# phymhan/pc-gan

Measured on AMD Instinct MI355X. Metric: images/sec (G+D step) 128x128 bs32 per GPU, higher is better.
Workload: dtype f32; 1 GPU; wsgan_emb UTKFace-shaped 128x128 bs32/GPU fp32: 9-block ResnetGenerator + 3-layer PatchGAN + ResNet-18 Elo encoder@224 + AlexNet IP@224, full optimize_parameters(); global_batch=32, parallelism=dp1

## Files before the change

pc-gan_amd/csrc/hgemm.hip:

```cpp
#include "igemm.h"

namespace pcgan {

typedef _Float16 f16x8 __attribute__((ext_vector_type(8)));
typedef _Float16 f16x4 __attribute__((ext_vector_type(4)));

typedef __bf16 bf16x8v __attribute__((ext_vector_type(8)));
typedef __bf16 bf16x4v __attribute__((ext_vector_type(4)));

template <int MODE, int BM, int BP, typename TA>
__global__ void __launch_bounds__(256) hgemm_kernel(IgemmArgs a) {
    static_assert(MODE == MODE_FWD_ZERO || MODE == MODE_FWD_REFLECT || MODE == MODE_BWD, "forward and plain data gradient");
    constexpr bool HALF = sizeof(TA) == 2;
    constexpr int NP = HALF ? 1 : 2;
    constexpr unsigned ES = sizeof(TA);
    constexpr int WM = (BM == 128 || (BM == 64 && BP == 64)) ? 2 : 1;
    constexpr int WP = 4 / WM;
    constexpr int WMT = BM / WM, WPT = BP / WP;
    constexpr int MI = WMT / 32, PJ = WPT / 32;
    constexpr int KPT = BP / 16;
    constexpr int ACH = BM * 4 / 256;
    constexpr int TROWS = NTAP_FWD + 1;
    constexpr int AH = BM + 8;
    __shared__ __attribute__((aligned(16))) f16x8 As[2][NP][2 * AH];
    __shared__ __attribute__((aligned(16))) f16x8 Bs[2][NP][2 * BP];
    __shared__ unsigned offT[TROWS][BP];
    __shared__ __attribute__((aligned(16))) float biasS[BM];
    __shared__ __attribute__((aligned(16))) float iswS[BM];

    const int nMt = (a.M + BM - 1) / BM;
    const int mt = blockIdx.x % nMt;
    int pt = blockIdx.x / nMt;
    int phase = 0;
    while (phase + 1 < a.nphase && pt >= a.tstart[phase + 1]) ++phase;
    pt -= a.tstart[phase];
    const PhaseArgs& P = a.ph[phase];
    const int tid = threadIdx.x;
    const int lane = tid & 63, lo = lane & 31, hi = lane >> 5;
    const int wave = __builtin_amdgcn_readfirstlane(tid >> 6);
    const int wm = wave / WP, wp = wave % WP;
    const int Ptot = P.Ptot, Kp = P.Kp;
    const int m0 = mt * BM, p0 = pt * BP;
    const int ph_nS = P.nS;
    const int T = P.nR * ph_nS;
    const int HgWg4 = a.Hg * a.Wg * (int)ES;
    const __amdgpu_buffer_rsrc_t rX = make_rsrc(a.X, a.x_bytes);
    const __amdgpu_buffer_rsrc_t rA = make_rsrc(P.A, (unsigned)a.M * (unsigned)Kp * 4u);

    float sx = 1.f;
    const int pl = tid % BP;
    {
        const int pg = p0 + pl;
        const bool pvalid = pg < Ptot;
        int gn = 0, py = 0, px = 0;
        if (pvalid) pix_coord(a, P, pg, gn, py, px);
        const unsigned vbase = (unsigned)gn * (unsigned)a.Cg * (unsigned)(a.Hg * a.Wg);
        for (int t = tid / BP; t <= T; t += 256 / BP) {
            const int ri = t / ph_nS, sj = t - ri * ph_nS;
            const int r = P.r0 + ri * a.tstep, sxx = P.s0 + sj * a.tstep;
            const bool live = pvalid && t < T;
            const unsigned y = axis_entry<MODE>(py, py + a.pad, true, r, a.Hg, a.sl, a.pad);
            const unsigned x = axis_entry<MODE>(px, px + a.pad, true, sxx, a.Wg, a.sl, a.pad);
            offT[t][pl] = (live && y != 0xffffffffu && x != 0xffffffffu) ? (vbase + y * (unsigned)a.Wg + x) * ES : OOB;
        }
    }
    const int ksub = __builtin_amdgcn_readfirstlane(tid / BP);
    __syncthreads();

    const int nst_all = Kp >> 4;
    const int nst_per = a.ksplit > 1 ? (nst_all + a.ksplit - 1) / a.ksplit : nst_all;
    const int st_begin = a.ksplit > 1 ? (int)blockIdx.z * nst_per : 0;
    const int st_end = st_begin + nst_per < nst_all ? st_begin + nst_per : nst_all;
    const int nst_here = st_end > st_begin ? st_end - st_begin : 0;

    int it_tap, it_c, it_k0, it_left = nst_here;
    {
        const int cc0 = st_begin / T;
        it_tap = st_begin - cc0 * T;
        it_c = cc0 * 16;
        it_k0 = st_begin * 16;
    }
    unsigned a_base[ACH];
#pragma unroll
    for (int j = 0; j < ACH; ++j) {
        const int q = tid + 256 * j;
        const int row = q >> 2, kc = (q & 3) * 4;
        a_base[j] = (m0 + row < a.M) ? (unsigned)((m0 + row) * Kp + kc) * 4u : OOB;
    }
    struct Stage {
        u32x4 av[ACH];
        unsigned bv[KPT];
    };
    auto load = [&](Stage& r) {
        const bool live = it_left > 0;
        const unsigned vo = offT[live ? it_tap : T][pl];
        const unsigned so = (unsigned)((it_c + ksub * KPT) * HgWg4);
#pragma unroll
        for (int j = 0; j < ACH; ++j) r.av[j] = __builtin_amdgcn_raw_buffer_load_b128(rA, live ? a_base[j] : OOB, (unsigned)it_k0 * 4u, 0);
#pragma unroll
        for (int i = 0; i < KPT; ++i) {
            if constexpr (HALF) r.bv[i] = (unsigned)__builtin_amdgcn_raw_buffer_load_b16(rX, vo, so + (unsigned)(i * HgWg4), 0);
            else r.bv[i] = __builtin_amdgcn_raw_buffer_load_b32(rX, vo, so + (unsigned)(i * HgWg4), 0);
        }
        --it_left;
        const int t1 = it_tap + 1;
        const bool wr = t1 == T;
        it_tap = wr ? 0 : t1;
        it_c += wr ? 16 : 0;
        it_k0 += 16;
    };
    auto stash = [&](const Stage& r, int buf) {
        if constexpr (HALF) {
#pragma unroll
            for (int j = 0; j < ACH; ++j) {
                const int q = tid + 256 * j;
                const int row = q >> 2, kc = (q & 3) * 4;
                bf16x4v h;
#pragma unroll
                for (int e = 0; e < 4; ++e) h[e] = (__bf16)__uint_as_float(r.av[j][e]);
                *reinterpret_cast<bf16x4v*>(reinterpret_cast<__bf16*>(&As[buf][0][(kc >> 3) * AH + row]) + (kc & 4)) = h;
            }
            typedef unsigned short usK __attribute__((ext_vector_type(KPT)));
            usK v;
#pragma unroll
            for (int e = 0; e < KPT; ++e) v[e] = (unsigned short)r.bv[e];
            if constexpr (KPT == 8) *reinterpret_cast<usK*>(&Bs[buf][0][ksub * BP + pl]) = v;
            else *reinterpret_cast<usK*>(reinterpret_cast<unsigned short*>(&Bs[buf][0][(ksub >> 1) * BP + pl]) + (ksub & 1) * 4) = v;
            return;
        }
#pragma unroll
        for (int j = 0; j < ACH; ++j) {
            const int q = tid + 256 * j;
            const int row = q >> 2, kc = (q & 3) * 4;
            typedef unsigned u32x2 __attribute__((ext_vector_type(2)));
            u32x2 h, l;
            h[0] = r.av[j][0]; h[1] = r.av[j][1];
            l[0] = r.av[j][2]; l[1] = r.av[j][3];
            _Float16* d0 = reinterpret_cast<_Float16*>(&As[buf][0][(kc >> 3) * AH + row]) + (kc & 4);
            _Float16* d1 = reinterpret_cast<_Float16*>(&As[buf][NP - 1][(kc >> 3) * AH + row]) + (kc & 4);
            *reinterpret_cast<u32x2*>(d0) = h;
            *reinterpret_cast<u32x2*>(d1) = l;
        }
        if constexpr (KPT == 8) {
            f16x8 h, l;
#pragma unroll
            for (int e = 0; e < 8; ++e) {
                _Float16 x, y;
                split2h(__uint_as_float(r.bv[e]) * sx, x, y);
                h[e] = x;
                l[e] = y;
            }
            Bs[buf][0][ksub * BP + pl] = h;
            Bs[buf][NP - 1][ksub * BP + pl] = l;
        } else {
            f16x4 h, l;
#pragma unroll
            for (int e = 0; e < 4; ++e) {
                _Float16 x, y;
                split2h(__uint_as_float(r.bv[e]) * sx, x, y);
                h[e] = x;
                l[e] = y;
            }
            *reinterpret_cast<f16x4*>(reinterpret_cast<_Float16*>(&Bs[buf][0][(ksub >> 1) * BP + pl]) + (ksub & 1) * 4) = h;
            *reinterpret_cast<f16x4*>(reinterpret_cast<_Float16*>(&Bs[buf][NP - 1][(ksub >> 1) * BP + pl]) + (ksub & 1) * 4) = l;
        }
    };

    f32x16 acc[MI][PJ];
#pragma unroll
    for (int i = 0; i < MI; ++i)
#pragma unroll
        for (int j = 0; j < PJ; ++j)
#pragma unroll
            for (int r = 0; r < 16; ++r) acc[i][j][r] = 0.f;
    struct Operands {
        f16x8 A[NP][MI], B[NP][PJ];
    };
    auto fetch = [&](Operands& o, int buf) {
#pragma unroll
        for (int p = 0; p < NP; ++p) {
#pragma unroll
            for (int i = 0; i < MI; ++i) o.A[p][i] = As[buf][p][hi * AH + wm * WMT + i * 32 + lo];
#pragma unroll
            for (int j = 0; j < PJ; ++j) o.B[p][j] = Bs[buf][p][hi * BP + wp * WPT + j * 32 + lo];
        }
    };
    auto mma = [&](const Operands& o) {
        if constexpr (HALF) {
#pragma unroll
            for (int i = 0; i < MI; ++i)
#pragma unroll
                for (int j = 0; j < PJ; ++j)
                    acc[i][j] = __builtin_amdgcn_mfma_f32_32x32x16_bf16(__builtin_bit_cast(bf16x8v, o.A[0][i]), __builtin_bit_cast(bf16x8v, o.B[0][j]),
                                                                         acc[i][j], 0, 0, 0);
            return;
        }
        constexpr int PA[3] = {NP - 1, 0, 0}, PB[3] = {0, NP - 1, 0};
#pragma unroll
        for (int q = 0; q < 3; ++q)
#pragma unroll
            for (int i = 0; i < MI; ++i)
#pragma unroll
                for (int j = 0; j < PJ; ++j)
                    acc[i][j] = __builtin_amdgcn_mfma_f32_32x32x16_f16(o.A[PA[q]][i], o.B[PB[q]][j], acc[i][j], 0, 0, 0);
    };
    auto interleave = [&]() {
        constexpr int NM = (HALF ? 1 : 3) * MI * PJ, NRD = NP * (MI + PJ);
#pragma unroll
        for (int q = 0; q < NM; ++q) {
            __builtin_amdgcn_sched_group_barrier(0x008, 1, 0);
            __builtin_amdgcn_sched_group_barrier(0x100, (NRD + NM - 1) / NM, 0);
            __builtin_amdgcn_sched_group_barrier(0x002, 48 / NM + 1, 0);
            __builtin_amdgcn_sched_group_barrier(0x200, 1, 0);
            __builtin_amdgcn_sched_group_barrier(0x020, (ACH + KPT + NM - 1) / NM, 0);
        }
    };

    Stage rg[2];
    if (nst_here > 0) {
        load(rg[0]);
        load(rg[1]);
    }
    if constexpr (!HALF) {
        const float m = thread_max_of_partials(a.x_amax, a.x_namax, tid, 256);
        sx = pow2_scale(block_max(m, biasS));
// ... 6 lines not shown
        Operands op[2];
        stash(rg[0], 0);
        __syncthreads();
        load(rg[0]);
        fetch(op[0], 0);
        stash(rg[1], 1);
        __syncthreads();
        load(rg[1]);
        const int nst2 = (nst_here + 1) & ~1;
        for (int s = 0; s < nst2; s += 2) {
#pragma unroll
            for (int t = 0; t < 2; ++t) {
                fetch(op[t ^ 1], t ^ 1);
                mma(op[t]);
                stash(rg[t], t);
                load(rg[t]);
                interleave();
                __builtin_amdgcn_sched_barrier(0);
                __syncthreads();
                __builtin_amdgcn_sched_barrier(0);
            }
        }
    }

    const float isx = 1.f / sx;
    const int YhYw = a.Yh * a.Yw;
    bool bad = false;
    if constexpr (!HALF) {
#pragma unroll
        for (int j = 0; j < PJ; ++j)
#pragma unroll
            for (int i = 0; i < MI; ++i)
#pragma unroll
                for (int r = 0; r < 16; ++r) bad |= is_nonfinite(acc[i][j][r]);
        report_nonfinite(a.ovf, bad);
    }
#pragma unroll
    for (int j = 0; j < PJ; ++j) {
        const int pix = p0 + wp * WPT + j * 32 + lo;
        if (pix >= Ptot) continue;
        int n, oy, ox;
        pix_coord(a, P, pix, n, oy, ox);
        if (a.ksplit > 1) {
            float* Yp = a.Ypart + ((size_t)blockIdx.z * a.N + n) * a.M * YhYw + oy * a.Yw + ox;
#pragma unroll
            for (int i = 0; i < MI; ++i)
#pragma unroll
                for (int r = 0; r < 16; ++r) {
                    const int ml = wm * WMT + i * 32 + (r & 3) + 8 * (r >> 2) + 4 * hi;
                    const int m = m0 + ml;
                    if (m < a.M) Yp[(size_t)m * YhYw] = (acc[i][j][r] * isx) * (HALF ? 1.f : iswS[ml]);
                }
            continue;
        }
        TA* Yp = (TA*)a.Y + (size_t)n * a.M * YhYw + oy * a.Yw + ox;
#pragma unroll
        for (int i = 0; i < MI; ++i)
#pragma unroll
            for (int r = 0; r < 16; ++r) {
                const int ml = wm * WMT + i * 32 + (r & 3) + 8 * (r >> 2) + 4 * hi;
                if (m0 + ml < a.M) st1(Yp + (size_t)(m0 + ml) * YhYw, act_apply((acc[i][j][r] * isx) * (HALF ? 1.f : iswS[ml]) + biasS[ml], a.act, a.slope));
            }
    }
}

template <int MODE>
static void launch_mode(const IgemmArgs& a, int bm, int bp, dim3 grid2, hipStream_t st) {
    if (bm == 128 && bp == 128) LAUNCH_TA(a.dtype, hgemm_kernel, grid2, a, MODE, 128, 128);
    else if (bm == 128) LAUNCH_TA(a.dtype, hgemm_kernel, grid2, a, MODE, 128, 64);
    else if (bp == 128) LAUNCH_TA(a.dtype, hgemm_kernel, grid2, a, MODE, 64, 128);
    else LAUNCH_TA(a.dtype, hgemm_kernel, grid2, a, MODE, 64, 64);
}
int launch_hgemm(int mode, const IgemmArgs& a, int bm, int bp, dim3 grid2, hipStream_t st) {
    switch (mode) {
        case MODE_FWD_ZERO: launch_mode<MODE_FWD_ZERO>(a, bm, bp, grid2, st); break;
        case MODE_FWD_REFLECT: launch_mode<MODE_FWD_REFLECT>(a, bm, bp, grid2, st); break;
        case MODE_BWD: launch_mode<MODE_BWD>(a, bm, bp, grid2, st); break;
        default: PCGAN_CHECK(false, "hgemm: no kernel for mode %d", mode);
    }
    PCGAN_LAUNCH_CHECK();
    return 0;
}

}

using namespace pcgan;

__global__ void __launch_bounds__(256) hgemm_presplit_kernel(float* __restrict__ A, int M, int Kp4, const float* __restrict__ rowmax) {
    const size_t n4 = (size_t)M * Kp4;
    for (size_t i = (size_t)blockIdx.x * 256 + threadIdx.x; i < n4; i += (size_t)gridDim.x * 256) {
        const float s = pow2_scale(rowmax[i / Kp4]);
        const float4 v = reinterpret_cast<const float4*>(A)[i];
        f16x4 h, l;
        _Float16 x, y;
        split2h(v.x * s, x, y); h[0] = x; l[0] = y;
        split2h(v.y * s, x, y); h[1] = x; l[1] = y;
        split2h(v.z * s, x, y); h[2] = x; l[2] = y;
        split2h(v.w * s, x, y); h[3] = x; l[3] = y;
        reinterpret_cast<f16x4*>(A)[2 * i] = h;
        reinterpret_cast<f16x4*>(A)[2 * i + 1] = l;
    }
}

int pcgan::launch_hgemm_presplit(float* A, int M, int Kp4, const float* rowmax, hipStream_t st) {
    hipLaunchKernelGGL(hgemm_presplit_kernel, dim3(capped_blocks((size_t)M * Kp4, 256, 2048)), dim3(256), 0, st, A, M, Kp4, rowmax);
    PCGAN_LAUNCH_CHECK();
    return 0;
}
```

pc-gan_amd/csrc/igemm.h:

```cpp
#pragma once
#include "common.h"
#include <type_traits>

namespace pcgan {

typedef float f32x16 __attribute__((ext_vector_type(16)));

enum { MODE_FWD_ZERO = 0, MODE_FWD_REFLECT = 1, MODE_BWD = 2, MODE_BWD_REFLECT = 3 };

typedef unsigned int u32x4 __attribute__((ext_vector_type(4)));
static constexpr unsigned OOB = 0x80000000u;

__device__ __forceinline__ __amdgpu_buffer_rsrc_t make_rsrc(const void* p, unsigned bytes) {
    return __builtin_amdgcn_make_buffer_rsrc(const_cast<void*>(p), 0, (int)bytes, 0x00020000);
}
__device__ __forceinline__ float ld_b32(__amdgpu_buffer_rsrc_t r, unsigned voff, unsigned soff) {
    return __uint_as_float(__builtin_amdgcn_raw_buffer_load_b32(r, voff, soff, 0));
}
__device__ __forceinline__ float4 ld_b128(__amdgpu_buffer_rsrc_t r, unsigned voff) {
    const u32x4 v = __builtin_amdgcn_raw_buffer_load_b128(r, voff, 0, 0);
    return make_float4(__uint_as_float(v.x), __uint_as_float(v.y), __uint_as_float(v.z), __uint_as_float(v.w));
}

template <typename TA>
// ... 115 lines not shown

struct Geom {
    int Hg, Wg, sl, pad;
};

template <int MODE>
__device__ __forceinline__ bool tap_offset(const Geom& a, int py, int px, int r, int s, int& off) {
    if (MODE == MODE_BWD || MODE == MODE_BWD_REFLECT) {
        const int ty = py + a.pad - r, tx = px + a.pad - s;
        const int oy = ty >> a.sl, ox = tx >> a.sl;
        off = oy * a.Wg + ox;
        return (ty >= 0) & (tx >= 0) & (oy < a.Hg) & (ox < a.Wg);
    } else {
        int iy = (py << a.sl) - a.pad + r;
        int ix = (px << a.sl) - a.pad + s;
        if (MODE == MODE_FWD_REFLECT) {
            iy = iy < 0 ? -iy : iy;
            iy = iy >= a.Hg ? 2 * (a.Hg - 1) - iy : iy;
            ix = ix < 0 ? -ix : ix;
            ix = ix >= a.Wg ? 2 * (a.Wg - 1) - ix : ix;
            off = iy * a.Wg + ix;
            return true;
        } else {
            off = iy * a.Wg + ix;
            return ((unsigned)iy < (unsigned)a.Hg) & ((unsigned)ix < (unsigned)a.Wg);
        }
    }
}

struct KIter {
    int ri, sj, c;
    __device__ __forceinline__ void advance(int n, int Cgp, int nS) {
        c += n;
        while (c >= Cgp) {
            c -= Cgp;
            if (++sj == nS) {
                sj = 0;
                ++ri;
            }
        }
    }
};

static constexpr int NTAP_FWD = 25;
static constexpr int NTAP_MIR = 9;
static constexpr int NTAP_CG4 = 49;

template <int MODE>
__device__ __forceinline__ unsigned axis_entry(int p, int base, bool base_ok, int tap, int n, int sl, int pad) {
    int i;
    bool ok;
    if (MODE == MODE_BWD || MODE == MODE_BWD_REFLECT) {
        const int t = base - tap;
        i = t >> sl;
        ok = base_ok & (t >= 0) & (i < n);
    } else {
        i = (p << sl) - pad + tap;
        if (MODE == MODE_FWD_REFLECT) {
            i = i < 0 ? -i : i;
            i = i >= n ? 2 * (n - 1) - i : i;
            ok = true;
        } else {
            ok = (unsigned)i < (unsigned)n;
        }
    }
    return ok ? (unsigned)i : 0xffffffffu;
}

__device__ __forceinline__ float4 ld_b128s(__amdgpu_buffer_rsrc_t r, unsigned voff, unsigned soff) {
    const u32x4 v = __builtin_amdgcn_raw_buffer_load_b128(r, voff, soff, 0);
    return make_float4(__uint_as_float(v.x), __uint_as_float(v.y), __uint_as_float(v.z), __uint_as_float(v.w));
}

__device__ __forceinline__ int refl_inner(int i, int n, int p) { return i == 0 ? 0 : (i == n - 2 * p - 1 ? n - 1 : i + p); }
__device__ __forceinline__ void pix_coord(const IgemmArgs& a, const PhaseArgs& P, int pg, int& n, int& py, int& px) {
    const int HsWs = P.Hs * P.Ws;
    n = pg / HsWs;
    const int rem = pg - n * HsWs;
    const int sy = rem / P.Ws;
    py = P.ymap ? refl_inner(sy, a.Yh, a.pad) : sy * a.ostep + P.fy;
    px = (rem - sy * P.Ws) * a.ostep + P.fx;
}

struct WgradArgs {
    const void* dY;
    const void* X;
    int dtype;
    float* Wp;
    int M, Kp, N, Cg, Cgp, Hg, Wg, Ho, Wo;
    int sl, pad, S;
    int magicS;
    int Ptot, chunks_per_split;
    unsigned x_bytes, dy_bytes;
};

static constexpr unsigned SM_INV = 0x40000000u;

static inline int round4(int v) { return (v + 3) & ~3; }
static inline size_t esz(const pcgan_conv_desc* d) { return d->dtype == PCGAN_BF16 ? 2 : 4; }

#define LAUNCH_TA(dt, KERNEL, GRID, ARG, ...)                                                                   \
    do {                                                                                                        \
        if ((dt) == PCGAN_BF16) hipLaunchKernelGGL((KERNEL<__VA_ARGS__, bf16>), GRID, dim3(256), 0, st, ARG);    \
        else hipLaunchKernelGGL((KERNEL<__VA_ARGS__, float>), GRID, dim3(256), 0, st, ARG);                      \
    } while (0)

void record_launch(int form, int mode, int bm, int bp, int ks, int nphase);
int launch_splitk_reduce(int dtype, hipStream_t st, const float* part, void* y, const float* bias, int ks, size_t out_elems, int M,
                         int HW, int act, float slope);

int launch_igemm_f32(int mode, const IgemmArgs& a, int bm, int bp, dim3 grid, dim3 grid2, hipStream_t st);
int launch_hgemm(int mode, const IgemmArgs& a, int bm, int bp, dim3 grid2, hipStream_t st);
int launch_hgemm_presplit(float* A, int M, int Kp4, const float* rowmax, hipStream_t st);
int launch_smallm(int mode, IgemmArgs& a, int pmax, hipStream_t st, float* part_ws, size_t part_bytes);
int launch_transpose4(const float* A, float* At, int M, int Kp, hipStream_t st);
int launch_pack_strip(const float* A, float* Ws, int M, int Cg, int Cgp, int nR, int nS, hipStream_t st);
int wgrad_splits(const pcgan_conv_desc* d, int* chunks_per_split);
int launch_wgrad(const pcgan_conv_desc* d, const WgradArgs& a, int splits, float* dw, int accumulate, hipStream_t st);

}
```

pc-gan_amd/csrc/igemm_conv.hip:

```cpp
#include "igemm.h"
#include <stdlib.h>
#include <mutex>

namespace pcgan {

template <typename TA>
__global__ void splitk_reduce_kernel(const float* __restrict__ part, TA* __restrict__ y, const float* __restrict__ bias,
                                     int ks, size_t n, int M, int HW, int act, float slope) {
    const size_t n4 = (n & 3) ? 0 : (n >> 2);
    const size_t stride = (size_t)gridDim.x * blockDim.x;
    for (size_t i = blockIdx.x * (size_t)blockDim.x + threadIdx.x; i < n4; i += stride) {
        float4 acc = reinterpret_cast<const float4*>(part)[i];
        for (int s = 1; s < ks; ++s) {
            const float4 v = reinterpret_cast<const float4*>(part + (size_t)s * n)[i];
            acc.x += v.x; acc.y += v.y; acc.z += v.z; acc.w += v.w;
        }
        float o[4] = {acc.x, acc.y, acc.z, acc.w};
#pragma unroll
        for (int u = 0; u < 4; ++u) {
            const size_t e = i * 4 + u;
            if (bias) o[u] += bias[(e / HW) % M];
            o[u] = act_apply(o[u], act, slope);
        }
        st4(y + 4 * i, make_float4(o[0], o[1], o[2], o[3]));
    }
    for (size_t e = (n4 << 2) + blockIdx.x * (size_t)blockDim.x + threadIdx.x; e < n; e += stride) {
        float acc = 0.f;
        for (int s = 0; s < ks; ++s) acc += part[(size_t)s * n + e];
        if (bias) acc += bias[(e / HW) % M];
        st1(y + e, act_apply(acc, act, slope));
    }
}

__global__ void repack_fwd_kernel(const float* __restrict__ w, float* __restrict__ A, int K, int C, int Cgp,
                                  int RS, int chunked) {
    const int Kp = RS * Cgp;
    const size_t total = (size_t)K * Kp;
    for (size_t i = blockIdx.x * (size_t)blockDim.x + threadIdx.x; i < total; i += (size_t)gridDim.x * blockDim.x) {
        const int k = (int)(i / Kp);
        const int j = (int)(i - (size_t)k * Kp);
        int tap, c;
        if (chunked) {
            const int t2 = j >> 4;
            const int cc = t2 / RS;
            tap = t2 - cc * RS;
            c = cc * 16 + (j & 15);
        } else {
            tap = j / Cgp;
            c = j - tap * Cgp;
        }
        A[i] = (c < C) ? w[((size_t)k * C + c) * RS + tap] : 0.f;
    }
}
__global__ void repack_bwd_kernel(const float* __restrict__ w, float* __restrict__ A, int K, int C, int Kgp,
                                  int R, int S, int r0, int s0, int tstep, int nR, int nS, int chunked, int fold) {
    const int Kp = nR * nS * Kgp;
    const size_t total = (size_t)C * Kp;
    for (size_t i = blockIdx.x * (size_t)blockDim.x + threadIdx.x; i < total; i += (size_t)gridDim.x * blockDim.x) {
        const int c = (int)(i / Kp);
        const int j = (int)(i - (size_t)c * Kp);
        int t, k;
        if (chunked) {
            const int t2 = j >> 4;
            const int kc = t2 / (nR * nS);
            t = t2 - kc * (nR * nS);
            k = kc * 16 + (j & 15);
        } else {
            t = j / Kgp;
            k = j - t * Kgp;
        }
        const int ri = t / nS, sj = t - ri * nS;
        const int r = r0 + ri * tstep, s = s0 + sj * tstep;
        float v = (k < K) ? w[(((size_t)k * C + c) * R + r) * S + s] : 0.f;
        if (k < K && fold == 1 && r == R - 1) v += w[(((size_t)k * C + c) * R + 0) * S + s];
        if (k < K && fold == 2 && r == 0) v += w[(((size_t)k * C + c) * R + (R - 1)) * S + s];
        A[i] = v;
    }
}

struct PackBwdArgs {
    const float* w;
    int K, C, Kgp, R, S, tstep, chunked, n;
    struct Entry {
        float* A;
        int r0, s0, nR, nS, fold;
    } e[16];
};
__global__ void repack_bwd_multi_kernel(PackBwdArgs a) {
    const PackBwdArgs::Entry& E = a.e[blockIdx.y];
    const int RS = E.nR * E.nS;
    const int Kp = RS * a.Kgp;
    const size_t total = (size_t)a.C * Kp;
    for (size_t i = blockIdx.x * (size_t)blockDim.x + threadIdx.x; i < total; i += (size_t)gridDim.x * blockDim.x) {
        const int c = (int)(i / Kp);
        const int j = (int)(i - (size_t)c * Kp);
        int t, k;
        if (a.chunked) {
            const int t2 = j >> 4;
            const int kc = t2 / RS;
            t = t2 - kc * RS;
            k = kc * 16 + (j & 15);
        } else {
            t = j / a.Kgp;
            k = j - t * a.Kgp;
        }
        const int ri = t / E.nS, sj = t - ri * E.nS;
        const int r = E.r0 + ri * a.tstep, sx = E.s0 + sj * a.tstep;
        float v = 0.f;
        if (k < a.K) {
            const float* wk = a.w + ((size_t)k * a.C + c) * a.R * a.S;
            v = wk[r * a.S + sx];
            if (E.fold == 1 && r == a.R - 1) v += wk[sx];
            if (E.fold == 2 && r == 0) v += wk[(a.R - 1) * a.S + sx];
        }
        E.A[i] = v;
    }
}

template <typename TA>
__global__ void reflect_fold_kernel(const TA* __restrict__ t, TA* __restrict__ dx, int NC, int H, int W,
                                    int pad, const float* __restrict__ bias, int C) {
    const int Hp = H + 2 * pad, Wp = W + 2 * pad;
    const int W4 = (W + 3) >> 2;
    const TA* tp = t + (size_t)blockIdx.y * Hp * Wp;
    TA* dp = dx + (size_t)blockIdx.y * H * W;
    const float bv = bias ? bias[blockIdx.y % C] : 0.f;
    for (int i = blockIdx.x * blockDim.x + threadIdx.x; i < H * W4; i += gridDim.x * blockDim.x) {
        const int y = i / W4, x0 = (i - y * W4) * 4;
        int ys[3], ny = 0;
        ys[ny++] = y + pad;
        if (y >= 1 && y <= pad) ys[ny++] = pad - y;
        if (y >= H - 1 - pad && y <= H - 2) ys[ny++] = pad + 2 * (H - 1) - y;
        float acc[4] = {0.f, 0.f, 0.f, 0.f};
        for (int a = 0; a < ny; ++a) {
            const TA* row = tp + ys[a] * Wp;
#pragma unroll
            for (int j = 0; j < 4; ++j) {
                const int x = x0 + j;
                if (x >= W) continue;
                float v = ld1(row + x + pad);
                if (x >= 1 && x <= pad) v += ld1(row + pad - x);
                if (x >= W - 1 - pad && x <= W - 2) v += ld1(row + pad + 2 * (W - 1) - x);
                acc[j] += v;
            }
        }
        if (bias) {
#pragma unroll
            for (int j = 0; j < 4; ++j) acc[j] += bv;
        }
        if ((W & 3) == 0) {
            st4(dp + y * W + x0, make_float4(acc[0], acc[1], acc[2], acc[3]));
        } else {
            for (int j = 0; j < 4 && x0 + j < W; ++j) st1(dp + y * W + x0 + j, acc[j]);
        }
    }
}

int launch_splitk_reduce(int dtype, hipStream_t st, const float* part, void* y, const float* bias, int ks, size_t out_elems, int M,
                         int HW, int act, float slope) {
    const dim3 b(capped_blocks(out_elems / 4, 256, 4096));
    if (dtype == PCGAN_BF16)
        hipLaunchKernelGGL(splitk_reduce_kernel<bf16>, b, dim3(256), 0, st, part, (bf16*)y, bias, ks, out_elems, M, HW, act, slope);
    else
        hipLaunchKernelGGL(splitk_reduce_kernel<float>, b, dim3(256), 0, st, part, (float*)y, bias, ks, out_elems, M, HW, act, slope);
    PCGAN_LAUNCH_CHECK();
    return 0;
}

static int check_desc(const pcgan_conv_desc* d) {
    PCGAN_CHECK(d != nullptr, "conv: null descriptor");
    PCGAN_CHECK(d->N > 0 && d->C > 0 && d->H > 0 && d->W > 0 && d->K > 0 && d->R > 0 && d->S > 0,
                "conv: non-positive dimension");
    PCGAN_CHECK(ilog2_exact(d->stride) >= 0 && d->stride <= 4, "conv: stride %d unsupported (1,2,4)", d->stride);
    PCGAN_CHECK(d->pad_mode == 0 || d->pad_mode == 1, "conv: pad_mode %d", d->pad_mode);
    PCGAN_CHECK(d->dtype == PCGAN_F32 || d->dtype == PCGAN_BF16, "conv: dtype %d (PCGAN_F32 / PCGAN_BF16)", d->dtype);
    const int P = (d->H + 2 * d->pad - d->R) / d->stride + 1, Q = (d->W + 2 * d->pad - d->S) / d->stride + 1;
    PCGAN_CHECK(P == d->P && Q == d->Q, "conv: output dims %dx%d do not match geometry %dx%d", d->P, d->Q, P, Q);
    if (d->pad_mode == 1)
        PCGAN_CHECK(d->pad < d->H && d->pad < d->W, "conv: reflection pad %d >= input size", d->pad);
    const size_t xin = (size_t)d->N * d->C * (d->H + 2 * d->pad) * (d->W + 2 * d->pad) * 4;
    const size_t yout = (size_t)d->N * d->K * d->P * d->Q * 4;
    PCGAN_CHECK(xin < (1ull << 31) && yout < (1ull << 31),
                "conv: tensor of %zu bytes exceeds the 2 GiB addressing limit of one launch (split the batch)",
                xin > yout ? xin : yout);
    PCGAN_CHECK((size_t)d->K * round4(d->C) * d->R * d->S * 4 < (1ull << 31) &&
                    (size_t)d->C * round4(d->K) * d->R * d->S * 4 < (1ull << 31), "conv: weight tensor too large");
    PCGAN_CHECK(d->R * d->S <= 512, "conv: filter too large");
    return 0;
}

static inline bool chunked_k(int Cg, int M, int R, int S) { return (Cg % 16) == 0 && M > 4 && R * S <= NTAP_FWD; }
static inline bool cg4_k(int Cg, int M, int R, int S) { return round4(Cg) == 4 && M > 4 && R * S <= NTAP_CG4; }
static inline long tile_blocks(int M, int ptot_max, int nphase, int mm, int pp) {
    return (long)((M + mm - 1) / mm) * ((ptot_max + pp - 1) / pp) * nphase;
}
static inline long split_below() { return 192; }
static inline bool may_split(int M, int ptot_max, int nphase) {
    if (option(OPT_HGEMM_KS) > 1) return M > 4;
// ... 221 lines not shown
}

struct BwdPhase {
    int fy, fx, r0, s0, nR, nS, Hs, Ws;
    int fold;
    size_t a_off, at_off, as_off;
};
struct BwdPlan {
    bool fused, rowfold, padded;
    int H, W, pad;
    bool need_zero;
    int n;
    BwdPhase ph[16];
};
static void bwd_plan(const pcgan_conv_desc* d, BwdPlan& pl) {
    memset(&pl, 0, sizeof(pl));
    pl.fused = bwd_fused_reflect(d);
    pl.rowfold = bwd_rowfold(d);
    pl.padded = d->pad_mode == 1 && !pl.fused;
    const int H = pl.H = pl.padded ? d->H + 2 * d->pad : d->H;
    const int W = pl.W = pl.padded ? d->W + 2 * d->pad : d->W;
    const int pad = pl.pad = pl.padded ? 0 : d->pad;
    const int stv = d->stride, Kgp = round4(d->K), RS = d->R * d->S;
    if (pl.rowfold) {
        for (int f = 0; f < 3; ++f) {
            BwdPhase& p = pl.ph[pl.n++];
            p.nR = d->R; p.nS = d->S; p.Ws = W; p.fold = f;
            p.Hs = f == 0 ? H - 2 : 1;
            p.fy = f == 0 ? 0 : (f == 1 ? 1 : H - 2);
            p.a_off = (size_t)f * d->C * RS * Kgp;
        }
        return;
    }
    size_t a_off = 0;
    size_t at_off = (size_t)d->C * RS * Kgp;
    size_t as_off = at_off + (size_t)RS * Kgp * 4;
    for (int fy = 0; fy < stv; ++fy) {
        for (int fx = 0; fx < stv; ++fx) {
            const int r0 = (fy + pad) % stv, s0 = (fx + pad) % stv;
            const int nR = r0 < d->R ? (d->R - r0 + stv - 1) / stv : 0;
            const int nS = s0 < d->S ? (d->S - s0 + stv - 1) / stv : 0;
            const int Hs = fy < H ? (H - fy + stv - 1) / stv : 0;
            const int Ws = fx < W ? (W - fx + stv - 1) / stv : 0;
            if (Hs * Ws == 0) continue;
            if (nR * nS == 0) {
                pl.need_zero = true;
                continue;
            }
            const BwdPhase p = {fy, fx, r0, s0, nR, nS, Hs, Ws, 0, a_off, at_off, as_off};
            pl.ph[pl.n++] = p;
            a_off += (size_t)d->C * nR * nS * Kgp;
            at_off += (size_t)nR * nS * Kgp * 4;
            as_off += (size_t)d->K * nS * 32;
        }
    }
}

static int pack_bwd(const pcgan_conv_desc* d, const BwdPlan& pl, const float* w, float* packed, hipStream_t st) {
    const int Kgp = round4(d->K);
    const int chunked = (int)chunked_k(d->K, d->C, d->R, d->S);
    if (d->C <= 4) {
        for (int i = 0; i < pl.n; ++i) {
            const BwdPhase& p = pl.ph[i];
            float* A = packed + p.a_off;
            const size_t total = (size_t)d->C * p.nR * p.nS * Kgp;
            hipLaunchKernelGGL(repack_bwd_kernel, dim3(capped_blocks(total, 256, 4096)), dim3(256), 0, st, w, A, d->K, d->C, Kgp, d->R,
                               d->S, p.r0, p.s0, d->stride, p.nR, p.nS, chunked, 0);
            PCGAN_LAUNCH_CHECK();
            if (int e = launch_transpose4(A, packed + p.at_off, d->C, p.nR * p.nS * Kgp, st)) return e;
            if (int e = launch_pack_strip(A, packed + p.as_off, d->C, d->K, Kgp, p.nR, p.nS, st)) return e;
        }
        return 0;
    }
    if (pl.n == 0) return 0;
    size_t max_total = 0;
    PackBwdArgs pk;
    memset(&pk, 0, sizeof(pk));
    pk.w = w; pk.K = d->K; pk.C = d->C; pk.Kgp = Kgp; pk.R = d->R; pk.S = d->S; pk.tstep = d->stride; pk.chunked = chunked; pk.n = pl.n;
    for (int i = 0; i < pl.n; ++i) {
        const BwdPhase& p = pl.ph[i];
        const size_t total = (size_t)d->C * p.nR * p.nS * Kgp;
        max_total = total > max_total ? total : max_total;
        PackBwdArgs::Entry& pe = pk.e[i];
        pe.A = packed + p.a_off; pe.r0 = p.r0; pe.s0 = p.s0; pe.nR = p.nR; pe.nS = p.nS; pe.fold = p.fold;
    }
    hipLaunchKernelGGL(repack_bwd_multi_kernel, dim3(capped_blocks(max_total, 256, 2048), pk.n), dim3(256), 0, st, pk);
    PCGAN_LAUNCH_CHECK();
    return 0;
}

static int conv2d_bwd_data_impl(const pcgan_conv_desc* d, const void* dy, const float* w, const float* packed,
                                const float* bias, void* dx, void* ws, size_t ws_bytes, pcgan_stream_t s, const HsplitOpt* hs = nullptr) {
    if (check_desc(d)) return 1;
    PCGAN_CHECK(dy && (w || packed), "conv2d_bwd_data: null pointer");
    PCGAN_CHECK(ws && ws_bytes >= pcgan_conv2d_workspace_bytes(d, PCGAN_PASS_BWD_DATA),
                "conv2d_bwd_data: workspace too small (%zu)", ws_bytes);
    PCGAN_CHECK(d->pad_mode == 0 || d->stride == 1, "conv2d_bwd_data: reflection padding needs stride 1");
    hipStream_t st = (hipStream_t)s;
    const int Kgp = round4(d->K), stv = d->stride;
    BwdPlan pl;
    bwd_plan(d, pl);
    float* Abase = packed ? const_cast<float*>(packed) : (float*)ws;
    if (!packed && pack_bwd(d, pl, w, Abase, st)) return 2;
    const size_t a_bytes = bwd_base_bytes(d);
    const int H = pl.H, W = pl.W;
    void* out = pl.padded ? (void*)((char*)ws + a_bytes) : dx;

    IgemmArgs a;
    memset(&a, 0, sizeof(a));
    a.X = dy; a.Y = out; a.dtype = d->dtype;
    a.bias = pl.padded ? nullptr : bias;
    a.M = d->C; a.N = d->N; a.Cg = d->K; a.Cgp = Kgp; a.Hg = d->P; a.Wg = d->Q;
    a.Yh = H; a.Yw = W;
    a.ostep = stv; a.sl = ilog2_exact(stv); a.pad = pl.pad; a.tstep = stv;
    a.act = PCGAN_ACT_NONE; a.slope = 0.f;
    a.chunked = chunked_k(d->K, d->C, d->R, d->S) ? 1 : (cg4_k(d->K, d->C, d->R, d->S) ? 2 : 0);
    a.rowfold = pl.rowfold;
    apply_hsplit(a, hs);
    a.x_bytes = (unsigned)((size_t)d->N * d->K * d->P * d->Q * esz(d));
    a.nphase = pl.n;
    for (int i = 0; i < pl.n; ++i) {
        const BwdPhase& q = pl.ph[i];
        PhaseArgs& p = a.ph[i];
        p.A = Abase + q.a_off; p.Kp = q.nR * q.nS * Kgp; p.Hs = q.Hs; p.Ws = q.Ws; p.fy = q.fy; p.fx = q.fx;
        if (d->C <= 4) {
            p.A = Abase + q.at_off;
            p.As = Abase + q.as_off;
        }
        p.r0 = q.r0; p.s0 = q.s0; p.nR = q.nR; p.nS = q.nS; p.Ptot = d->N * q.Hs * q.Ws;
        p.ymap = pl.rowfold && q.fold == 0;
    }
    if (pl.rowfold) return launch_igemm(MODE_BWD_REFLECT, a, st, nullptr, 0);
    if (pl.need_zero) {
        PCGAN_CHECK(!bias, "conv2d_bwd_data: bias with uncovered phases is unsupported");
        hipError_t e = hipMemsetAsync(out, 0, (size_t)d->N * d->C * H * W * esz(d), st);
        PCGAN_CHECK(e == hipSuccess, "memset failed: %s", hipGetErrorString(e));
    }
    float* part = (bwd_part_bytes(d) && !pl.padded && !pl.need_zero) ? (float*)((char*)ws + a_bytes) : nullptr;
    if (launch_igemm(pl.fused ? MODE_BWD_REFLECT : MODE_BWD, a, st, part, bwd_part_bytes(d))) return 2;
    if (pl.padded) return pcgan::launch_reflect_fold(out, dx, d->N * d->C, d->H, d->W, d->pad, d->dtype, st, bias, d->C);
    return 0;
}

extern "C" int pcgan_conv2d_bwd_data(const pcgan_conv_desc* d, const void* dy, const float* w,
                                     const float* bias, void* dx, void* ws, size_t ws_bytes,
                                     pcgan_stream_t s) {
    if (check_desc(d)) return 1;
    PCGAN_CHECK(w && dx, "conv2d_bwd_data: null pointer");
    return conv2d_bwd_data_impl(d, dy, w, nullptr, bias, dx, ws, ws_bytes, s);
}
extern "C" int pcgan_conv2d_bwd_data_packed(const pcgan_conv_desc* d, const void* dy, const float* packed,
                                            const float* bias, void* dx, void* ws, size_t ws_bytes,
                                            pcgan_stream_t s) {
    if (check_desc(d)) return 1;
    PCGAN_CHECK(packed && dx, "conv2d_bwd_data_packed: null pointer");
    pcgan::TimerScope timer(pcgan::timer_kind_res(d, pcgan::TIMER_RES_DGRAD), (hipStream_t)s);
    return conv2d_bwd_data_impl(d, dy, nullptr, packed, bias, dx, ws, ws_bytes, s);
}

extern "C" int pcgan_conv2d_hgemm_supported(const pcgan_conv_desc* d, int pass) {
    if (!d || d->dtype != PCGAN_F32) return 0;
    if (pass == PCGAN_PASS_FWD) return chunked_k(d->C, d->K, d->R, d->S) && d->K > 32;
    if (pass == PCGAN_PASS_BWD_DATA) return d->pad_mode == 0 && chunked_k(d->K, d->C, d->R, d->S) && d->C > 32;
    return 0;
}
extern "C" int pcgan_conv2d_fwd_packed_hsplit(const pcgan_conv_desc* d, const void* x, const float* x_amax, int n_amax, const float* packed,
                                              const float* w_amax, const float* bias, void* y, int act, float slope, void* ws,
                                              size_t ws_bytes, pcgan_stream_t s) {
    if (check_desc(d)) return 1;
    PCGAN_CHECK(pcgan_conv2d_hgemm_supported(d, PCGAN_PASS_FWD), "conv2d_fwd_packed_hsplit: unsupported shape");
    PCGAN_CHECK(packed && x_amax && n_amax > 0 && w_amax, "conv2d_fwd_packed_hsplit: null pointer");
    const HsplitOpt hs = {x_amax, n_amax, w_amax};
    return conv2d_fwd_impl(d, x, nullptr, packed, bias, y, act, slope, ws, ws_bytes, s, &hs);
}
extern "C" int pcgan_conv2d_bwd_data_packed_hsplit(const pcgan_conv_desc* d, const void* dy, const float* dy_amax, int n_amax,
                                                   const float* packed, const float* w_amax, const float* bias, void* dx, void* ws,
                                                   size_t ws_bytes, pcgan_stream_t s) {
    if (check_desc(d)) return 1;
    PCGAN_CHECK(pcgan_conv2d_hgemm_supported(d, PCGAN_PASS_BWD_DATA), "conv2d_bwd_data_packed_hsplit: unsupported shape");
    PCGAN_CHECK(packed && dx && dy_amax && n_amax > 0 && w_amax, "conv2d_bwd_data_packed_hsplit: null pointer");
    const HsplitOpt hs = {dy_amax, n_amax, w_amax};
    return conv2d_bwd_data_impl(d, dy, nullptr, packed, bias, dx, ws, ws_bytes, s, &hs);
}

extern "C" int pcgan_conv2d_hgemm_pack(const pcgan_conv_desc* d, int pass, const float* w, float* w_rowmax, float* packed,
                                       pcgan_stream_t s) {
    if (check_desc(d)) return 1;
    PCGAN_CHECK(pcgan_conv2d_hgemm_supported(d, pass), "conv2d_hgemm_pack: unsupported shape or pass");
    PCGAN_CHECK(w && w_rowmax && packed, "conv2d_hgemm_pack: null pointer");
    hipStream_t st = (hipStream_t)s;
    const bool fwd = pass == PCGAN_PASS_FWD;
    const int M = fwd ? d->K : d->C, RS = d->R * d->S;
    if (launch_weight_row_absmax(w, d->K, d->C, RS, fwd ? 0 : 1, w_rowmax, st)) return 2;
    if (pcgan_conv2d_pack_weights(d, pass, w, packed, s)) return 1;
    if (fwd) return launch_hgemm_presplit(packed, M, RS * round4(d->C) / 4, w_rowmax, st);
    BwdPlan pl;
    bwd_plan(d, pl);
    for (int i = 0; i < pl.n; ++i)
        if (int e = launch_hgemm_presplit(packed + pl.ph[i].a_off, M, pl.ph[i].nR * pl.ph[i].nS * round4(d->K) / 4, w_rowmax, st)) return e;
    return 0;
}

extern "C" int pcgan_igemm_last_launch(int* info, int n) {
    PCGAN_CHECK(info != nullptr && n > 0, "igemm_last_launch: null output");
    std::lock_guard<std::mutex> lk(g_launch_mu);
    for (int i = 0; i < n; ++i) info[i] = i < PCGAN_IGEMM_LAUNCH_INFO ? g_launch[i] : 0;
    return 0;
}

extern "C" size_t pcgan_conv2d_packed_bytes(const pcgan_conv_desc* d, int pass) {
    if (!d) return 0;
    if (pass == PCGAN_PASS_FWD) return fwd_base_bytes(d);
    if (pass == PCGAN_PASS_BWD_DATA) return bwd_base_bytes(d);
    return 0;
}
extern "C" int pcgan_conv2d_pack_weights(const pcgan_conv_desc* d, int pass, const float* w, float* packed,
                                         pcgan_stream_t s) {
    if (check_desc(d)) return 1;
    PCGAN_CHECK(w && packed, "conv2d_pack_weights: null pointer");
    if (pass == PCGAN_PASS_FWD) return pack_fwd(d, w, packed, (hipStream_t)s);
    PCGAN_CHECK(pass == PCGAN_PASS_BWD_DATA, "conv2d_pack_weights: pass %d has no packed weights", pass);
    PCGAN_CHECK(d->pad_mode == 0 || d->stride == 1, "conv2d_bwd_data: reflection padding needs stride 1");
    BwdPlan pl;
    bwd_plan(d, pl);
    return pack_bwd(d, pl, w, packed, (hipStream_t)s);
}

extern "C" int pcgan_conv2d_bwd_weight(const pcgan_conv_desc* d, const void* x, const void* dy, float* dw,
                                       int accumulate, void* ws, size_t ws_bytes, pcgan_stream_t s) {
    if (check_desc(d)) return 1;
    PCGAN_CHECK(x && dy && dw, "conv2d_bwd_weight: null pointer");
    PCGAN_CHECK(ws && ws_bytes >= pcgan_conv2d_workspace_bytes(d, PCGAN_PASS_BWD_WEIGHT),
                "conv2d_bwd_weight: workspace too small (%zu)", ws_bytes);
    hipStream_t st = (hipStream_t)s;
    pcgan::TimerScope timer(pcgan::timer_kind_res(d, pcgan::TIMER_RES_WGRAD), st);
    const int Cgp = round4(d->C), RS = d->R * d->S;
    WgradArgs a;
    memset(&a, 0, sizeof(a));
    a.dY = dy; a.X = x; a.Wp = (float*)ws; a.dtype = d->dtype;
    a.M = d->K; a.Kp = RS * Cgp; a.N = d->N; a.Cg = d->C; a.Cgp = Cgp;
    a.Hg = d->H; a.Wg = d->W; a.Ho = d->P; a.Wo = d->Q;
    a.sl = ilog2_exact(d->stride); a.pad = d->pad; a.S = d->S;
    a.magicS = (65536 + d->S - 1) / d->S;
    a.Ptot = d->N * d->P * d->Q;
    a.x_bytes = (unsigned)((size_t)d->N * d->C * d->H * d->W * esz(d));
    a.dy_bytes = (unsigned)((size_t)d->N * d->K * d->P * d->Q * esz(d));
    const int splits = wgrad_splits(d, &a.chunks_per_split);
    return launch_wgrad(d, a, splits, dw, accumulate, st);
}
```

Measured before the change: 1210 images/sec.

## Pack hgemm weights in LDS-native row-block layout and fuse pack with split

Weights for the split-fp16 hgemm path are now packed directly from the original tensor into a row-block layout that matches shared memory, so each wave loads contiguous 16-byte chunks and stores them straight into LDS without the per-element scatter into hi/lo planes. The separate pack and presplit kernels are merged into one pack kernel, removing one pass over the packed weights. The A-matrix addressing in the kernel changes from a per-row K offset to a per-stage block stride, which depends on the packed layout and the kernel agreeing exactly, and may break for tail blocks or ksplit.

```diff
diff --git a/pc-gan_amd/csrc/hgemm.hip b/pc-gan_amd/csrc/hgemm.hip
--- a/pc-gan_amd/csrc/hgemm.hip
+++ b/pc-gan_amd/csrc/hgemm.hip
@@ -4,6 +4,8 @@
 
 typedef _Float16 f16x8 __attribute__((ext_vector_type(8)));
 typedef _Float16 f16x4 __attribute__((ext_vector_type(4)));
+
+static constexpr int HGEMM_RB = 64;
 
 typedef __bf16 bf16x8v __attribute__((ext_vector_type(8)));
 typedef __bf16 bf16x4v __attribute__((ext_vector_type(4)));
@@ -73,19 +75,28 @@
     const int st_end = st_begin + nst_per < nst_all ? st_begin + nst_per : nst_all;
     const int nst_here = st_end > st_begin ? st_end - st_begin : 0;
 
-    int it_tap, it_c, it_k0, it_left = nst_here;
+    int it_tap, it_c, it_st, it_left = nst_here;
     {
         const int cc0 = st_begin / T;
         it_tap = st_begin - cc0 * T;
         it_c = cc0 * 16;
-        it_k0 = st_begin * 16;
+        it_st = st_begin;
     }
     unsigned a_base[ACH];
+    int a_st[ACH];
 #pragma unroll
     for (int j = 0; j < ACH; ++j) {
-        const int q = tid + 256 * j;
-        const int row = q >> 2, kc = (q & 3) * 4;
-        a_base[j] = (m0 + row < a.M) ? (unsigned)((m0 + row) * Kp + kc) * 4u : OOB;
+        if constexpr (HALF) {
+            const int q = tid + 256 * j;
+            const int row = q >> 2, kc = (q & 3) * 4;
+            a_base[j] = (m0 + row < a.M) ? (unsigned)((m0 + row) * Kp + kc) * 4u : OOB;
+            a_st[j] = 64;
+        } else {
+            const int mb0 = m0 + HGEMM_RB * j;
+            const int rb = a.M - mb0 < HGEMM_RB ? a.M - mb0 : HGEMM_RB;
+            a_base[j] = lane < rb ? (unsigned)(mb0 * Kp) * 4u + (unsigned)(wave * rb + lane) * 16u : OOB;
+            a_st[j] = rb > 0 ? rb * 64 : 0;
+        }
     }
     struct Stage {
         u32x4 av[ACH];
@@ -96,7 +107,7 @@
         const unsigned vo = offT[live ? it_tap : T][pl];
         const unsigned so = (unsigned)((it_c + ksub * KPT) * HgWg4);
 #pragma unroll
-        for (int j = 0; j < ACH; ++j) r.av[j] = __builtin_amdgcn_raw_buffer_load_b128(rA, live ? a_base[j] : OOB, (unsigned)it_k0 * 4u, 0);
+        for (int j = 0; j < ACH; ++j) r.av[j] = __builtin_amdgcn_raw_buffer_load_b128(rA, live ? a_base[j] : OOB, (unsigned)(it_st * a_st[j]), 0);
 #pragma unroll
         for (int i = 0; i < KPT; ++i) {
             if constexpr (HALF) r.bv[i] = (unsigned)__builtin_amdgcn_raw_buffer_load_b16(rX, vo, so + (unsigned)(i * HgWg4), 0);
@@ -107,7 +118,7 @@
         const bool wr = t1 == T;
         it_tap = wr ? 0 : t1;
         it_c += wr ? 16 : 0;
-        it_k0 += 16;
+        ++it_st;
     };
     auto stash = [&](const Stage& r, int buf) {
         if constexpr (HALF) {
@@ -129,18 +140,8 @@
             return;
         }
 #pragma unroll
-        for (int j = 0; j < ACH; ++j) {
-            const int q = tid + 256 * j;
-            const int row = q >> 2, kc = (q & 3) * 4;
-            typedef unsigned u32x2 __attribute__((ext_vector_type(2)));
-            u32x2 h, l;
-            h[0] = r.av[j][0]; h[1] = r.av[j][1];
-            l[0] = r.av[j][2]; l[1] = r.av[j][3];
-            _Float16* d0 = reinterpret_cast<_Float16*>(&As[buf][0][(kc >> 3) * AH + row]) + (kc & 4);
-            _Float16* d1 = reinterpret_cast<_Float16*>(&As[buf][NP - 1][(kc >> 3) * AH + row]) + (kc & 4);
-            *reinterpret_cast<u32x2*>(d0) = h;
-            *reinterpret_cast<u32x2*>(d1) = l;
-        }
+        for (int j = 0; j < ACH; ++j)
+            *reinterpret_cast<u32x4*>(&As[buf][(wave >> 1) * (NP - 1)][(wave & 1) * AH + HGEMM_RB * j + lane]) = r.av[j];
         if constexpr (KPT == 8) {
             f16x8 h, l;
 #pragma unroll
@@ -313,28 +314,53 @@
     return 0;
 }
 
-}
-
-using namespace pcgan;
-
-__global__ void __launch_bounds__(256) hgemm_presplit_kernel(float* __restrict__ A, int M, int Kp4, const float* __restrict__ rowmax) {
-    const size_t n4 = (size_t)M * Kp4;
-    for (size_t i = (size_t)blockIdx.x * 256 + threadIdx.x; i < n4; i += (size_t)gridDim.x * 256) {
-        const float s = pow2_scale(rowmax[i / Kp4]);
-        const float4 v = reinterpret_cast<const float4*>(A)[i];
-        f16x4 h, l;
-        _Float16 x, y;
-        split2h(v.x * s, x, y); h[0] = x; l[0] = y;
-        split2h(v.y * s, x, y); h[1] = x; l[1] = y;
-        split2h(v.z * s, x, y); h[2] = x; l[2] = y;
-        split2h(v.w * s, x, y); h[3] = x; l[3] = y;
-        reinterpret_cast<f16x4*>(A)[2 * i] = h;
-        reinterpret_cast<f16x4*>(A)[2 * i + 1] = l;
-    }
-}
-
-int pcgan::launch_hgemm_presplit(float* A, int M, int Kp4, const float* rowmax, hipStream_t st) {
-    hipLaunchKernelGGL(hgemm_presplit_kernel, dim3(capped_blocks((size_t)M * Kp4, 256, 2048)), dim3(256), 0, st, A, M, Kp4, rowmax);
+struct HpackFwd {
+    const float* w;
+    int C, RS;
+    __device__ __forceinline__ float at(int m, int j) const { return pack_fwd_at(w, C, C, RS, 1, m, j); }
+};
+struct HpackBwd {
+    const float* w;
+    int K, C, R, S, tstep;
+    PackBwdTaps taps;
+    __device__ __forceinline__ float at(int m, int j) const { return pack_bwd_at(w, K, C, K, R, S, tstep, 1, taps, m, j); }
+};
+template <typename SRC>
+__global__ void __launch_bounds__(256) hgemm_pack_kernel(SRC src, float* __restrict__ A, int M, int Kp, const float* __restrict__ rowmax) {
+    const int mb0 = (int)blockIdx.y * HGEMM_RB;
+    const int rb = M - mb0 < HGEMM_RB ? M - mb0 : HGEMM_RB;
+    f16x8* blk = reinterpret_cast<f16x8*>(A + (size_t)mb0 * Kp);
+    const int n = rb * (Kp >> 3);
+    for (int t = (int)blockIdx.x * 256 + (int)threadIdx.x; t < n; t += (int)gridDim.x * 256) {
+        const int hs = t / rb, row = t - hs * rb;
+        const int m = mb0 + row;
+        const float s = pow2_scale(rowmax[m]);
+        f16x8 h, l;
+#pragma unroll
+        for (int e = 0; e < 8; ++e) {
+            _Float16 x, y;
+            split2h(src.at(m, hs * 8 + e) * s, x, y);
+            h[e] = x;
+            l[e] = y;
+        }
+        const int u = ((hs >> 1) * 4 + (hs & 1)) * rb + row;
+        blk[u] = h;
+        blk[u + 2 * rb] = l;
+    }
+}
+template <typename SRC>
+static int launch_hgemm_pack(const SRC& src, float* A, int M, int Kp, const float* rowmax, hipStream_t st) {
+    const dim3 grid(capped_blocks((size_t)HGEMM_RB * (Kp >> 3), 256, 256), (unsigned)((M + HGEMM_RB - 1) / HGEMM_RB));
+    hipLaunchKernelGGL(hgemm_pack_kernel<SRC>, grid, dim3(256), 0, st, src, A, M, Kp, rowmax);
     PCGAN_LAUNCH_CHECK();
     return 0;
 }
+int launch_hgemm_pack_fwd(const float* w, float* A, int K, int C, int RS, const float* rowmax, hipStream_t st) {
+    return launch_hgemm_pack(HpackFwd{w, C, RS}, A, K, RS * C, rowmax, st);
+}
+int launch_hgemm_pack_bwd(const float* w, float* A, int K, int C, int R, int S, int tstep, const PackBwdTaps& taps, const float* rowmax,
+                          hipStream_t st) {
+    return launch_hgemm_pack(HpackBwd{w, K, C, R, S, tstep, taps}, A, C, taps.nR * taps.nS * K, rowmax, st);
+}
+
+}
diff --git a/pc-gan_amd/csrc/igemm.h b/pc-gan_amd/csrc/igemm.h
--- a/pc-gan_amd/csrc/igemm.h
+++ b/pc-gan_amd/csrc/igemm.h
@@ -221,6 +221,48 @@
     px = (rem - sy * P.Ws) * a.ostep + P.fx;
 }
 
+__device__ __forceinline__ float pack_fwd_at(const float* __restrict__ w, int C, int Cgp, int RS, int chunked, int k, int j) {
+    int tap, c;
+    if (chunked) {
+        const int t2 = j >> 4;
+        const int cc = t2 / RS;
+        tap = t2 - cc * RS;
+        c = cc * 16 + (j & 15);
+    } else {
+        tap = j / Cgp;
+        c = j - tap * Cgp;
+    }
+    return (c < C) ? w[((size_t)k * C + c) * RS + tap] : 0.f;
+}
+struct PackBwdTaps {
+    int r0, s0, nR, nS;
+    int fold;
+};
+__device__ __forceinline__ float pack_bwd_at(const float* __restrict__ w, int K, int C, int Kgp, int R, int S, int tstep, int chunked,
+                                             const PackBwdTaps& E, int c, int j) {
+    const int RS = E.nR * E.nS;
+    int t, k;
+    if (chunked) {
+        const int t2 = j >> 4;
+        const int kc = t2 / RS;
+        t = t2 - kc * RS;
+        k = kc * 16 + (j & 15);
+    } else {
+        t = j / Kgp;
+        k = j - t * Kgp;
+    }
+    const int ri = t / E.nS, sj = t - ri * E.nS;
+    const int r = E.r0 + ri * tstep, s = E.s0 + sj * tstep;
+    float v = 0.f;
+    if (k < K) {
+        const float* wk = w + ((size_t)k * C + c) * R * S;
+        v = wk[r * S + s];
+        if (E.fold == 1 && r == R - 1) v += wk[s];
+        if (E.fold == 2 && r == 0) v += wk[(R - 1) * S + s];
+    }
+    return v;
+}
+
 struct WgradArgs {
     const void* dY;
     const void* X;
@@ -250,7 +292,9 @@
 
 int launch_igemm_f32(int mode, const IgemmArgs& a, int bm, int bp, dim3 grid, dim3 grid2, hipStream_t st);
 int launch_hgemm(int mode, const IgemmArgs& a, int bm, int bp, dim3 grid2, hipStream_t st);
-int launch_hgemm_presplit(float* A, int M, int Kp4, const float* rowmax, hipStream_t st);
+int launch_hgemm_pack_fwd(const float* w, float* A, int K, int C, int RS, const float* rowmax, hipStream_t st);
+int launch_hgemm_pack_bwd(const float* w, float* A, int K, int C, int R, int S, int tstep, const PackBwdTaps& taps, const float* rowmax,
+                          hipStream_t st);
 int launch_smallm(int mode, IgemmArgs& a, int pmax, hipStream_t st, float* part_ws, size_t part_bytes);
 int launch_transpose4(const float* A, float* At, int M, int Kp, hipStream_t st);
 int launch_pack_strip(const float* A, float* Ws, int M, int Cg, int Cgp, int nR, int nS, hipStream_t st);
diff --git a/pc-gan_amd/csrc/igemm_conv.hip b/pc-gan_amd/csrc/igemm_conv.hip
--- a/pc-gan_amd/csrc/igemm_conv.hip
+++ b/pc-gan_amd/csrc/igemm_conv.hip
@@ -39,42 +39,18 @@
     for (size_t i = blockIdx.x * (size_t)blockDim.x + threadIdx.x; i < total; i += (size_t)gridDim.x * blockDim.x) {
         const int k = (int)(i / Kp);
         const int j = (int)(i - (size_t)k * Kp);
-        int tap, c;
-        if (chunked) {
-            const int t2 = j >> 4;
-            const int cc = t2 / RS;
-            tap = t2 - cc * RS;
-            c = cc * 16 + (j & 15);
-        } else {
-            tap = j / Cgp;
-            c = j - tap * Cgp;
-        }
-        A[i] = (c < C) ? w[((size_t)k * C + c) * RS + tap] : 0.f;
+        A[i] = pack_fwd_at(w, C, Cgp, RS, chunked, k, j);
     }
 }
 __global__ void repack_bwd_kernel(const float* __restrict__ w, float* __restrict__ A, int K, int C, int Kgp,
                                   int R, int S, int r0, int s0, int tstep, int nR, int nS, int chunked, int fold) {
     const int Kp = nR * nS * Kgp;
     const size_t total = (size_t)C * Kp;
+    const PackBwdTaps E = {r0, s0, nR, nS, fold};
     for (size_t i = blockIdx.x * (size_t)blockDim.x + threadIdx.x; i < total; i += (size_t)gridDim.x * blockDim.x) {
         const int c = (int)(i / Kp);
         const int j = (int)(i - (size_t)c * Kp);
-        int t, k;
-        if (chunked) {
-            const int t2 = j >> 4;
-            const int kc = t2 / (nR * nS);
-            t = t2 - kc * (nR * nS);
-            k = kc * 16 + (j & 15);
-        } else {
-            t = j / Kgp;
-            k = j - t * Kgp;
-        }
-        const int ri = t / nS, sj = t - ri * nS;
-        const int r = r0 + ri * tstep, s = s0 + sj * tstep;
-        float v = (k < K) ? w[(((size_t)k * C + c) * R + r) * S + s] : 0.f;
-        if (k < K && fold == 1 && r == R - 1) v += w[(((size_t)k * C + c) * R + 0) * S + s];
-        if (k < K && fold == 2 && r == 0) v += w[(((size_t)k * C + c) * R + (R - 1)) * S + s];
-        A[i] = v;
+        A[i] = pack_bwd_at(w, K, C, Kgp, R, S, tstep, chunked, E, c, j);
     }
 }
 
@@ -83,37 +59,17 @@
     int K, C, Kgp, R, S, tstep, chunked, n;
     struct Entry {
         float* A;
-        int r0, s0, nR, nS, fold;
+        PackBwdTaps taps;
     } e[16];
 };
 __global__ void repack_bwd_multi_kernel(PackBwdArgs a) {
     const PackBwdArgs::Entry& E = a.e[blockIdx.y];
-    const int RS = E.nR * E.nS;
-    const int Kp = RS * a.Kgp;
+    const int Kp = E.taps.nR * E.taps.nS * a.Kgp;
     const size_t total = (size_t)a.C * Kp;
     for (size_t i = blockIdx.x * (size_t)blockDim.x + threadIdx.x; i < total; i += (size_t)gridDim.x * blockDim.x) {
         const int c = (int)(i / Kp);
         const int j = (int)(i - (size_t)c * Kp);
-        int t, k;
-        if (a.chunked) {
-            const int t2 = j >> 4;
-            const int kc = t2 / RS;
-            t = t2 - kc * RS;
-            k = kc * 16 + (j & 15);
-        } else {
-            t = j / a.Kgp;
-            k = j - t * a.Kgp;
-        }
-        const int ri = t / E.nS, sj = t - ri * E.nS;
-        const int r = E.r0 + ri * a.tstep, sx = E.s0 + sj * a.tstep;
-        float v = 0.f;
-        if (k < a.K) {
-            const float* wk = a.w + ((size_t)k * a.C + c) * a.R * a.S;
-            v = wk[r * a.S + sx];
-            if (E.fold == 1 && r == a.R - 1) v += wk[sx];
-            if (E.fold == 2 && r == 0) v += wk[(a.R - 1) * a.S + sx];
-        }
-        E.A[i] = v;
+        E.A[i] = pack_bwd_at(a.w, a.K, a.C, a.Kgp, a.R, a.S, a.tstep, a.chunked, E.taps, c, j);
     }
 }
 
@@ -501,7 +457,7 @@
         const size_t total = (size_t)d->C * p.nR * p.nS * Kgp;
         max_total = total > max_total ? total : max_total;
         PackBwdArgs::Entry& pe = pk.e[i];
-        pe.A = packed + p.a_off; pe.r0 = p.r0; pe.s0 = p.s0; pe.nR = p.nR; pe.nS = p.nS; pe.fold = p.fold;
+        pe.A = packed + p.a_off; pe.taps = PackBwdTaps{p.r0, p.s0, p.nR, p.nS, p.fold};
     }
     hipLaunchKernelGGL(repack_bwd_multi_kernel, dim3(capped_blocks(max_total, 256, 2048), pk.n), dim3(256), 0, st, pk);
     PCGAN_LAUNCH_CHECK();
@@ -609,14 +565,17 @@
     PCGAN_CHECK(w && w_rowmax && packed, "conv2d_hgemm_pack: null pointer");
     hipStream_t st = (hipStream_t)s;
     const bool fwd = pass == PCGAN_PASS_FWD;
-    const int M = fwd ? d->K : d->C, RS = d->R * d->S;
+    const int RS = d->R * d->S;
     if (launch_weight_row_absmax(w, d->K, d->C, RS, fwd ? 0 : 1, w_rowmax, st)) return 2;
-    if (pcgan_conv2d_pack_weights(d, pass, w, packed, s)) return 1;
-    if (fwd) return launch_hgemm_presplit(packed, M, RS * round4(d->C) / 4, w_rowmax, st);
+    if (fwd) return launch_hgemm_pack_fwd(w, packed, d->K, d->C, RS, w_rowmax, st);
     BwdPlan pl;
     bwd_plan(d, pl);
-    for (int i = 0; i < pl.n; ++i)
-        if (int e = launch_hgemm_presplit(packed + pl.ph[i].a_off, M, pl.ph[i].nR * pl.ph[i].nS * round4(d->K) / 4, w_rowmax, st)) return e;
+    for (int i = 0; i < pl.n; ++i) {
+        const BwdPhase& p = pl.ph[i];
+        if (int e = launch_hgemm_pack_bwd(w, packed + p.a_off, d->K, d->C, d->R, d->S, d->stride, PackBwdTaps{p.r0, p.s0, p.nR, p.nS, p.fold},
+                                          w_rowmax, st))
+            return e;
+    }
     return 0;
 }
 
```

Result: no change. 1218 images/sec (median of 6 runs) (+0.6%).
